# davidbau/rewriting

Measured on AMD Instinct MI355X. Metric: images/sec StyleGANv2-1024 fwd, higher is better.
Workload: dtype f32 (conv operands split into exact f16 pairs from 32x32 up, f32 accumulate); 1 GPU; stylegan2-1024 generator forward (FFHQ-1024 architecture); batch_per_gpu=64, mconv=seq, weights=synthetic seed 0, parallelism=seeds partitioned per rank, no collective, matrix_mode=split, direct_sums=auto

## Files before the change

### rewriting_amd/csrc/rw_dconv.hip

```cpp
#include "rw_common.h"
#include <stdlib.h>
typedef float dc_f32x4 __attribute__((ext_vector_type(4)));
typedef float dc_f32x2 __attribute__((ext_vector_type(2)));
typedef unsigned dc_u32x4 __attribute__((ext_vector_type(4)));
typedef int dc_i32x4 __attribute__((ext_vector_type(4)));
typedef _Float16 dc_f16x2 __attribute__((ext_vector_type(2)));
typedef _Float16 dc_f16x8 __attribute__((ext_vector_type(8)));

struct DconvProblem {
  const float* x; const unsigned char* wp; float* y;
  const float* style; const float* demod; const float* noise; const float* noise_w; const float* bias; int act;
  const float* post;
  const float* rgb_weight; const float* rgb_style; const float* rgb_bias; const float* rgb_skip; float* rgb_out;
  float rgb_scale;
  int batch, in_ch, out_ch, h, w;
  int tiles_x, tiles_y, o_tiles;
  int strided;
  float w_scale;
  float u_inv;
  const float* x_amax; float* y_amax;
};

#ifndef DC_ABL
#define DC_ABL 0
// ... 59 lines not shown
  constexpr int BUFB = NPIX * 64;
  constexpr int VCH = 32 * WM;
  __shared__ __attribute__((aligned(16))) unsigned char Ls[2 * BUFB];
  __shared__ __attribute__((aligned(16))) float St[512];
  __shared__ float Ct[2][VCH];
  __shared__ float Cr[3][(RGB || RGBP) ? 32 * WM : 1];
  __shared__ float Red[4];

  const int tid = threadIdx.x, lane = tid & 63;
  const int wave = __builtin_amdgcn_readfirstlane(tid >> 6);
  const int wm = wave / WN, wn = wave % WN;
  const int lk = lane >> 4, lt = lane & 15;

  const int local = dc_xcd_remap(blockIdx.x, gridDim.x);
  const int ot = local % p.o_tiles;
  int pg = local / p.o_tiles;
  const int tx = pg % p.tiles_x; pg /= p.tiles_x;
  const int ty = pg % p.tiles_y;
  const int ib = pg / p.tiles_y;
  const int y0 = ty * TR, x0 = tx * 32;
  const int64_t hw = (int64_t)p.h * p.w;
  const int NC = p.in_ch >> 4, T = 9 * NC;
  const int real_ch = UP ? p.out_ch >> 2 : p.out_ch;

  float in_scale, out_scale;
  {
    float smax = p.style ? 0.f : 1.f;
    if (p.style)
      for (int i = tid; i < p.in_ch; i += 256) smax = fmaxf(smax, fabsf(p.style[(int64_t)ib * p.in_ch + i]));
    smax = rw_wave_max(smax);
    if (lane == 0) Red[wave] = smax;
    __syncthreads();
    smax = fmaxf(fmaxf(Red[0], Red[1]), fmaxf(Red[2], Red[3]));
    const float am = rw_bound_load(p.x_amax) * smax;
    int e = (int)((__float_as_uint(am) >> 23) & 0xff) - 126;
    e = e < -100 ? -100 : (e > 100 ? 100 : e);
    in_scale = __uint_as_float((unsigned)(127 + 14 - e) << 23);
    out_scale = __uint_as_float((unsigned)(127 + e - 14) << 23) * p.u_inv;
  }
  const float gain = p.act ? 1.4142135623730951f : 1.f, slope = p.act ? 0.2f : 1.f;
  for (int i = tid; i < p.in_ch; i += 256) St[i] = (p.style ? p.style[(int64_t)ib * p.in_ch + i] : 1.0f) * in_scale;
  if (tid < VCH) {
    const int o = UP ? 16 * ot + (tid & 15) : ot * VCH + tid;
    Ct[0][tid] = (p.demod ? p.demod[(int64_t)ib * real_ch + o] * p.w_scale : p.w_scale) * out_scale * gain;
    Ct[1][tid] = p.act ? p.bias[o] * gain : 0.f;
    if (RGB || RGBP) {
      const float sr = p.rgb_scale * p.rgb_style[(int64_t)ib * p.out_ch + o];
#pragma unroll
      for (int cc = 0; cc < 3; ++cc) Cr[cc][tid] = sr * p.rgb_weight[cc * p.out_ch + o];
    }
  }
  const float noise_wg = p.noise ? p.noise_w[0] * gain : 0.f;
  __syncthreads();

  const __amdgpu_buffer_rsrc_t xsrc = __builtin_amdgcn_make_buffer_rsrc(
      const_cast<float*>(p.x + (int64_t)ib * p.in_ch * hw), 0, (int)((int64_t)p.in_ch * hw * 4), 0x00020000);
  const int hw4 = (int)hw * 4;
  int xoff[SI], loff[SI];
#pragma unroll
  for (int s = 0; s < SI; ++s) {
    const int pi = 64 * s + lane;
    const int r = pi / DC_PW, cc = pi - r * DC_PW;
    const int iy = y0 - 1 + r, ix = x0 - 1 + cc;
    const bool ok = pi < NPIX && iy >= 0 && iy < p.h && ix >= 0 && ix < p.w;
    xoff[s] = ok ? (iy * p.w + ix) * 4 : 0x7fffffff;
    loff[s] = pi < NPIX ? pi * 64 + ((wave ^ dc_swz(cc)) << 4) : -1;
  }
  constexpr int SH = (SI + 1) / 2;
  float raw[SH][4];
  auto stage_load = [&](int c, auto half_tag) __attribute__((always_inline)) {
    constexpr int S0 = decltype(half_tag)::value ? SH : 0, S1 = decltype(half_tag)::value ? SI : SH;
    const int s0 = (16 * c + 4 * wave) * hw4;
#pragma unroll
    for (int s = S0; s < S1; ++s)
#pragma unroll
      for (int k = 0; k < 4; ++k)
        raw[s - S0][k] = (DC_ABL & 1) ? 1.f : __uint_as_float(__builtin_amdgcn_raw_buffer_load_b32(xsrc, xoff[s], s0 + k * hw4, 0));
  };
  auto stage_store = [&](int c, int buf, auto half_tag) __attribute__((always_inline)) {
    constexpr int S0 = decltype(half_tag)::value ? SH : 0, S1 = decltype(half_tag)::value ? SI : SH;
    const dc_f32x4 sv = *reinterpret_cast<const dc_f32x4*>(&St[16 * c + 4 * wave]);
    unsigned char* dst = Ls + buf * BUFB;
#pragma unroll
    for (int s = S0; s < S1; ++s) {
      const float (&rw)[4] = raw[s - S0];
      const float v0 = rw[0] * sv[0], v1 = rw[1] * sv[1], v2 = rw[2] * sv[2], v3 = rw[3] * sv[3];
      const dc_f16x2 h01 = __builtin_convertvector(dc_f32x2{v0, v1}, dc_f16x2);
      const dc_f16x2 h23 = __builtin_convertvector(dc_f32x2{v2, v3}, dc_f16x2);
      float r0, r1, r2, r3;
      asm("v_fma_mix_f32 %0, -%1, 1.0, %2 op_sel_hi:[1,0,0]" : "=v"(r0) : "v"(h01), "v"(v0));
      asm("v_fma_mix_f32 %0, -%1, 1.0, %2 op_sel:[1,0,0] op_sel_hi:[1,0,0]" : "=v"(r1) : "v"(h01), "v"(v1));
      asm("v_fma_mix_f32 %0, -%1, 1.0, %2 op_sel_hi:[1,0,0]" : "=v"(r2) : "v"(h23), "v"(v2));
      asm("v_fma_mix_f32 %0, -%1, 1.0, %2 op_sel:[1,0,0] op_sel_hi:[1,0,0]" : "=v"(r3) : "v"(h23), "v"(v3));
      const dc_f16x2 l01 = __builtin_convertvector(dc_f32x2{r0, r1}, dc_f16x2);
      const dc_f16x2 l23 = __builtin_convertvector(dc_f32x2{r2, r3}, dc_f16x2);
      const dc_f16x8 word = {h01[0], h01[1], h23[0], h23[1], l01[0], l01[1], l23[0], l23[1]};
      if (loff[s] >= 0) *reinterpret_cast<dc_f16x8*>(dst + loff[s]) = word;
    }
  };

  const int vb0 = ot * (2 * WM) + 2 * wm;
  const unsigned char* wbase = p.wp + (int64_t)vb0 * T * 1024 + lane * 8;
  dc_f16x8 W[3][2][2];
  dc_f32x2 Wc[3][2][2];
  auto wload = [&](int ky, int t) __attribute__((always_inline)) {
#pragma unroll
    for (int ob = 0; ob < 2; ++ob)
#pragma unroll
      for (int part = 0; part < 2; ++part) {
        if (DC_ABL & 4) Wc[ky][ob][part] = dc_f32x2{1.f, 1.f};
        else Wc[ky][ob][part] = *reinterpret_cast<const dc_f32x2*>(wbase + ((int64_t)ob * T + t) * 1024 + part * 512);
      }
  };
  auto wexpand = [&](int ky) __attribute__((always_inline)) {
#pragma unroll
    for (int ob = 0; ob < 2; ++ob) {
      W[ky][ob][0] = dc_expand(Wc[ky][ob][0]);
      if (DC_PRODUCTS == 4 || ky == 2) W[ky][ob][1] = dc_expand(Wc[ky][ob][1]);
      else if (ky == 1) W[0][ob][1] = dc_pair(Wc[0][ob][1], Wc[1][ob][1]);
    }
  };

  dc_f32x4 acc[2][8];
#pragma unroll
  for (int ob = 0; ob < 2; ++ob)
#pragma unroll
    for (int pb = 0; pb < 8; ++pb) acc[ob][pb] = dc_f32x4{0.f, 0.f, 0.f, 0.f};

  unsigned bbase[3];
#pragma unroll
  for (int kx = 0; kx < 3; ++kx) {
    const int cc = lt + kx;
    bbase[kx] = (unsigned)((4 * wn * DC_PW + cc) * 64 + ((lk ^ dc_swz(cc)) << 4));
  }
  auto bread = [&](const unsigned char* lb, int kx, int idx) __attribute__((always_inline)) {
    return *reinterpret_cast<const dc_f16x8*>(lb + bbase[kx] + ((idx >> 1) * DC_PW + 16 * (idx & 1)) * 64);
  };

  auto chunk = [&](int c, auto last_tag) __attribute__((always_inline)) {
    constexpr bool LAST = decltype(last_tag)::value != 0;
    const int buf = c & 1;
    const unsigned char* lb = Ls + buf * BUFB;
    if (!LAST) stage_load(c + 1, rw_int<0>());
    dc_f16x8 bcur = bread(lb, 0, 0);
    dc_f16x8 bprev[2] = {bcur, bcur};
#pragma unroll
    for (int kx = 0; kx < 3; ++kx) {
      const bool more = !LAST || kx < 2;
      const int tn = kx < 2 ? 9 * c + kx + 1 : 9 * (c + 1);
#pragma unroll
      for (int idx = 0; idx < 12; ++idx) {
        const int r = idx >> 1, half = idx & 1;
        if (half == 0 && r < 3) wexpand(r);
        dc_f16x8 bnext = bcur;
        if (idx + 1 < 12) bnext = bread(lb, kx, idx + 1);
        else if (kx < 2) bnext = bread(lb, kx + 1, 0);
#pragma unroll
        for (int ky = 0; ky < 3; ++ky) {
          const int pr = r - ky;
          if (pr < 0 || pr > 3) continue;
          const int pb = 2 * pr + half;
          if (DC_ABL & 2) { asm volatile("" :: "v"(bcur), "v"(W[ky][0][0]), "v"(W[ky][0][1]), "v"(W[ky][1][0]), "v"(W[ky][1][1])); continue; }
          acc[0][pb] = __builtin_amdgcn_mfma_f32_16x16x32_f16(bcur, W[ky][0][0], acc[0][pb], 0, 0, 0);
          acc[1][pb] = __builtin_amdgcn_mfma_f32_16x16x32_f16(bcur, W[ky][1][0], acc[1][pb], 0, 0, 0);
          if (DC_PRODUCTS == 4 || ky == 2) {
            acc[0][pb] = __builtin_amdgcn_mfma_f32_16x16x32_f16(bcur, W[ky][0][1], acc[0][pb], 0, 0, 0);
            acc[1][pb] = __builtin_amdgcn_mfma_f32_16x16x32_f16(bcur, W[ky][1][1], acc[1][pb], 0, 0, 0);
          }
        }
        if (DC_PRODUCTS == 3 && r >= 1 && r <= 4 && !(DC_ABL & 2)) {
          const int pb = 2 * (r - 1) + half;
          const dc_f16x8 hh = dc_pair(bprev[half], bcur);
          acc[0][pb] = __builtin_amdgcn_mfma_f32_16x16x32_f16(hh, W[0][0][1], acc[0][pb], 0, 0, 0);
          acc[1][pb] = __builtin_amdgcn_mfma_f32_16x16x32_f16(hh, W[0][1][1], acc[1][pb], 0, 0, 0);
        }
        bprev[half] = bcur;
        __builtin_amdgcn_sched_barrier(0);
        if (more && half == 1 && r >= 3) wload(r - 3, tn + 3 * (r - 3));
        bcur = bnext;
      }
      if (!LAST && kx == 0) {
        stage_store(c + 1, buf ^ 1, rw_int<0>());
        stage_load(c + 1, rw_int<1>());
      }
      __builtin_amdgcn_sched_barrier(0);
    }
    if (!LAST) {
      stage_store(c + 1, buf ^ 1, rw_int<1>());
      __syncthreads();
    }
  };

  wload(0, 0);
  wload(1, 3);
  wload(2, 6);
  stage_load(0, rw_int<0>());
  stage_store(0, 0, rw_int<0>());
  stage_load(0, rw_int<1>());
  stage_store(0, 0, rw_int<1>());
  __syncthreads();

  for (int c = 0; c + 1 < NC; ++c) chunk(c, rw_int<0>());
  chunk(NC - 1, rw_int<1>());
  if (DC_ABL & 8) { if (acc[0][0][0] != 12345.f) return; }

  float ymax = 0.f;
  if (MODE == 0 || RGBP) {
    const int oc = 16 * (2 * wm) + lt;
    const float sc[2] = {Ct[0][oc], Ct[0][oc + 16]}, bs[2] = {Ct[1][oc], Ct[1][oc + 16]};
    float* yb = p.y + ((int64_t)ib * p.out_ch + ot * VCH + oc) * hw;
    float cr[2][3] = {{0.f, 0.f, 0.f}, {0.f, 0.f, 0.f}};
    float* rb = nullptr;
    if (RGBP) {
#pragma unroll
      for (int ob = 0; ob < 2; ++ob)
#pragma unroll
        for (int cc = 0; cc < 3; ++cc) cr[ob][cc] = Cr[cc][oc + 16 * ob];
      rb = p.rgb_out + (((int64_t)(ot * WM + wm) * p.batch + ib) * 3 + (lt < 3 ? lt : 0)) * hw;
    }
#pragma unroll
    for (int pb = 0; pb < 8; ++pb) {
      const int64_t pix = (int64_t)(y0 + 4 * wn + (pb >> 1)) * p.w + x0 + 16 * (pb & 1) + 4 * lk;
      dc_f32x4 nz = {0.f, 0.f, 0.f, 0.f};
      if (p.noise) nz = *reinterpret_cast<const dc_f32x4*>(p.noise + (int64_t)ib * hw + pix) * noise_wg;
      dc_f32x4 v[2];
#pragma unroll
      for (int ob = 0; ob < 2; ++ob) {
#pragma unroll
        for (int j = 0; j < 4; ++j) {
          const float u = acc[ob][pb][j] * sc[ob] + nz[j] + bs[ob];
          v[ob][j] = fmaxf(u, u * slope);
          ymax = fmaxf(ymax, fabsf(v[ob][j]));
        }
        *reinterpret_cast<dc_f32x4*>(yb + (int64_t)(16 * ob) * hw + pix) = v[ob];
      }
      if (RGBP) {
        dc_f32x4 sum[3];
#pragma unroll
        for (int j = 0; j < 4; ++j)
#pragma unroll
          for (int cc = 0; cc < 3; ++cc) sum[cc][j] = dc_row_sum(v[0][j] * cr[0][cc] + v[1][j] * cr[1][cc]);
        if (lt < 3) *reinterpret_cast<dc_f32x4*>(rb + pix) = lt == 0 ? sum[0] : (lt == 1 ? sum[1] : sum[2]);
      }
    }
  } else if (UP) {
    const float sc = Ct[0][lt], bs = Ct[1][lt];
    const int ch = 16 * ot + lt;
    const float post = p.post ? p.post[(int64_t)ib * real_ch + ch] : 1.f;
    const int W2 = 2 * p.w;
    const int64_t hw2 = 4 * hw;
    float* yb = p.y + ((int64_t)ib * real_ch + ch) * hw2;
#pragma unroll
    for (int pb = 0; pb < 8; ++pb) {
      const int64_t pix = (int64_t)(2 * (y0 + 4 * wn + (pb >> 1)) + wm) * W2 + 2 * (x0 + 16 * (pb & 1) + 4 * lk);
      dc_f32x4 n0 = {0.f, 0.f, 0.f, 0.f}, n1 = n0;
      if (p.noise) {
        const float* np = p.noise + (int64_t)ib * hw2 + pix;
        n0 = *reinterpret_cast<const dc_f32x4*>(np) * noise_wg;
        n1 = *reinterpret_cast<const dc_f32x4*>(np + 4) * noise_wg;
      }
      dc_f32x4 q0 = {acc[0][pb][0], acc[1][pb][0], acc[0][pb][1], acc[1][pb][1]};
      dc_f32x4 q1 = {acc[0][pb][2], acc[1][pb][2], acc[0][pb][3], acc[1][pb][3]};
#pragma unroll
      for (int k = 0; k < 4; ++k) {
        const float u0 = q0[k] * sc + n0[k] + bs, u1 = q1[k] * sc + n1[k] + bs;
        q0[k] = fmaxf(u0, u0 * slope) * post; q1[k] = fmaxf(u1, u1 * slope) * post;
        ymax = fmaxf(ymax, fmaxf(fabsf(q0[k]), fabsf(q1[k])));
      }
      *reinterpret_cast<dc_f32x4*>(yb + pix) = q0;
      *reinterpret_cast<dc_f32x4*>(yb + pix + 4) = q1;
    }
  } else {
    const float sc[2] = {Ct[0][lt], Ct[0][lt + 16]}, bs[2] = {Ct[1][lt], Ct[1][lt + 16]};
    float cr[2][3];
#pragma unroll
    for (int ob = 0; ob < 2; ++ob)
#pragma unroll
      for (int cc = 0; cc < 3; ++cc) cr[ob][cc] = Cr[cc][lt + 16 * ob];
#pragma unroll
    for (int pb = 0; pb < 8; ++pb) {
      const int64_t pix = (int64_t)(y0 + 4 * wn + (pb >> 1)) * p.w + x0 + 16 * (pb & 1) + 4 * lk;
      dc_f32x4 nz = {0.f, 0.f, 0.f, 0.f};
      if (p.noise) nz = *reinterpret_cast<const dc_f32x4*>(p.noise + (int64_t)ib * hw + pix) * noise_wg;
      dc_f32x4 sum[3];
#pragma unroll
      for (int j = 0; j < 4; ++j) {
        float u0 = acc[0][pb][j] * sc[0] + nz[j] + bs[0], u1 = acc[1][pb][j] * sc[1] + nz[j] + bs[1];
        u0 = fmaxf(u0, u0 * slope); u1 = fmaxf(u1, u1 * slope);
#pragma unroll
        for (int cc = 0; cc < 3; ++cc) sum[cc][j] = dc_row_sum(u0 * cr[0][cc] + u1 * cr[1][cc]);
      }
      if (lt < 3) {
        const dc_f32x4 mine = lt == 0 ? sum[0] : (lt == 1 ? sum[1] : sum[2]);
        const int64_t off = ((int64_t)ib * 3 + lt) * hw + pix;
        dc_f32x4 o4 = mine + (p.rgb_bias ? p.rgb_bias[lt] : 0.f);
        if (p.rgb_skip) o4 += *reinterpret_cast<const dc_f32x4*>(p.rgb_skip + off);
        *reinterpret_cast<dc_f32x4*>(p.rgb_out + off) = o4;
      }
    }
  }
  if (!RGB && p.y_amax) rw_bound_store_wave(p.y_amax, rw_wave_max(ymax));
}

template <int MODE, int WM, int MW, int NL, int WC>
__device__ __forceinline__ void dconv_ws_body(const DconvProblem& p) {
  constexpr bool UP = MODE == 1, RGB = MODE == 2, RGBP = MODE == 3, PLAIN = MODE == 0 || MODE == 3;
  static_assert(!RGB || WM == 1, "ToRGB: one wave holds all out-channels of its pixels");
  static_assert(!UP || WM == 2, "UP: the wave pairs are the two row phases");
  constexpr int WN = MW / WM, WR = WN / WC, TR = 4 * WR, PR = TR + 2, TC = 32 * WC, PW = TC + 2;
  static_assert(WR * WC == WN && WR >= 1, "strips tile the workgroup's pixels");
  constexpr int QW = 4 / NL, NLL = 64 * NL;
  constexpr int NPIX = PR * PW, BUFB = NPIX * 64;
  constexpr int IPR = TC / 4 + 2, NITEM = PR * IPR, SI = (NITEM + 63) / 64;
  constexpr int VCH = 32 * WM;
  constexpr int WBUF = 2 * WM * 9 * 1024;
  __shared__ __attribute__((aligned(16))) unsigned char Ls[2 * BUFB];
  __shared__ __attribute__((aligned(16))) unsigned char Wl[2 * WBUF];
  __shared__ float Ct[2][2][VCH];
  __shared__ float Cr[2][3][VCH];
  __shared__ float Po[2][16];

  const int tid = threadIdx.x, lane = tid & 63;
  const int wave = __builtin_amdgcn_readfirstlane(tid >> 6);
  const int64_t hw = (int64_t)p.h * p.w;
  const int NC = p.in_ch >> 4, T = 9 * NC;
  const int real_ch = UP ? p.out_ch >> 2 : p.out_ch;
  const float gain = p.act ? 1.4142135623730951f : 1.f, slope = p.act ? 0.2f : 1.f;

  const int64_t total = (int64_t)p.batch * p.tiles_y * p.tiles_x * p.o_tiles;
  const int per = (int)((total + gridDim.x - 1) / gridDim.x);
  const int bx = p.strided ? dc_xcd_remap(blockIdx.x, gridDim.x) : blockIdx.x;
  const int t0 = p.strided ? 0 : bx * per;
  const int t1 = p.strided ? (int)((total - bx + gridDim.x - 1) / gridDim.x)
                           : (int)((int64_t)t0 + per < total ? t0 + per : total);
  if (t0 >= t1) {
    if (!RGB && p.y_amax) rw_bound_store_wave(p.y_amax, 0.f);
    return;
  }
  const int N = (t1 - t0) * NC;
  const int t_mul = p.strided ? gridDim.x : 1, t_add = p.strided ? bx : 0;
  auto decode = [&](int pos, int& ot, int& tx, int& ty, int& ib) __attribute__((always_inline)) {
    const int tile = pos * t_mul + t_add;
    ot = tile % p.o_tiles;
    int pg = tile / p.o_tiles;
    tx = pg % p.tiles_x; pg /= p.tiles_x;
    ty = pg % p.tiles_y;
    ib = pg / p.tiles_y;
  };
  auto lds_barrier = [&]() __attribute__((always_inline)) {
    asm volatile("" ::: "memory");
    __builtin_amdgcn_s_waitcnt(0xC07F);
    __builtin_amdgcn_s_barrier();
    asm volatile("" ::: "memory");
  };

  if (wave >= MW) {
    const int g2 = QW * (wave - MW), lid = (wave - MW) * 64 + lane;
    const float xam = rw_bound_load(p.x_amax);
    const int hw4 = (int)hw * 4;
    int loff[SI];
#pragma unroll
    for (int s = 0; s < SI; ++s) {
      const int it = 64 * s + lane;
      const int r = it / IPR, j = it - r * IPR;
      loff[s] = it < NITEM ? (r * PW + 4 * j - 3) * 64 : -1000000;
    }
    int l_tile = t0, l_c = 0, l_ib = -1, l_ot = 0, l_y0 = 0, l_x0 = 0;
    float in_scale = 1.f, out_scale = 1.f;
    int xoff[SI];
    __amdgpu_buffer_rsrc_t xsrc = __builtin_amdgcn_make_buffer_rsrc(const_cast<float*>(p.x), 0, 0, 0x00020000);
    dc_f32x4 raw[QW][SI][4];
    float psv[QW][4];
    float a_demod = 1.f, a_bias = 0.f, a_rgb = 0.f, a_post = 1.f, a_oscale = 1.f, a_iscale = 1.f;
    float a_crw[3] = {0.f, 0.f, 0.f};
    bool a_first = false;
    int a_par = 0;
    float crw[3] = {0.f, 0.f, 0.f};
    if (RGB && lid < 32) {
#pragma unroll
      for (int cc = 0; cc < 3; ++cc) crw[cc] = p.rgb_weight[cc * p.out_ch + lid] * p.rgb_scale;
    }

    float sv[QW][4];
    int l_s0 = 0;
    const unsigned char* l_wsrc = p.wp;
    auto setup = [&]() __attribute__((always_inline)) {
      if (l_tile >= t1) { l_tile = t1 - 1; l_c = NC - 1; }
      a_first = l_c == 0;
      if (l_c == 0) {
        int tx, ty, ib;
        decode(l_tile, l_ot, tx, ty, ib);
        l_y0 = ty * TR; l_x0 = tx * TC;
        if (ib != l_ib) {
          l_ib = ib;
          float smax = 0.f;
          for (int i = lane; i < p.in_ch; i += 64) smax = fmaxf(smax, fabsf(p.style[(int64_t)ib * p.in_ch + i]));
          smax = rw_wave_max(smax);
          const float am = xam * smax;
          int e = (int)((__float_as_uint(am) >> 23) & 0xff) - 126;
          e = e < -100 ? -100 : (e > 100 ? 100 : e);
          in_scale = __uint_as_float((unsigned)(127 + 14 - e) << 23);
          out_scale = __uint_as_float((unsigned)(127 + e - 14) << 23) * p.u_inv;
          xsrc = __builtin_amdgcn_make_buffer_rsrc(const_cast<float*>(p.x + (int64_t)ib * p.in_ch * hw), 0,
                                                   (int)((int64_t)p.in_ch * hw * 4), 0x00020000);
        }
#pragma unroll
        for (int s = 0; s < SI; ++s) {
          const int it = 64 * s + lane;
          const int r = it / IPR, j = it - r * IPR;
          const int iy = l_y0 - 1 + r, ix = l_x0 - 4 + 4 * j;
          const bool ok = it < NITEM && iy >= 0 && iy < p.h && ix >= 0 && ix < p.w;
          xoff[s] = ok ? (iy * p.w + ix) * 4 : 0x7ffffff0;
        }
        a_par = (l_tile - t0) & 1;
        a_oscale = out_scale;
        if (lid < VCH) {
          const int o = UP ? 16 * l_ot + (lid & 15) : l_ot * VCH + lid;
          a_demod = p.demod ? p.demod[(int64_t)l_ib * real_ch + o] : 1.f;
          a_bias = p.act ? p.bias[o] : 0.f;
          if (RGB || RGBP) a_rgb = p.rgb_style[(int64_t)l_ib * p.out_ch + o];
          if (RGBP) {
#pragma unroll
            for (int cc = 0; cc < 3; ++cc) a_crw[cc] = p.rgb_weight[cc * p.out_ch + o] * p.rgb_scale;
          }
          if (UP && lid < 16 && p.post) a_post = p.post[(int64_t)l_ib * real_ch + o];
        }
      }
#pragma unroll
      for (int q = 0; q < QW; ++q)
#pragma unroll
        for (int k = 0; k < 4; ++k) psv[q][k] = p.style[(int64_t)l_ib * p.in_ch + 16 * l_c + 4 * (g2 + q) + k];
      a_iscale = in_scale;
      l_s0 = (16 * l_c + 4 * g2) * hw4;
      l_wsrc = p.wp + ((int64_t)(l_ot * (2 * WM) + (wave - MW)) * T + 9 * l_c) * 1024;
      if (++l_c == NC) { l_c = 0; ++l_tile; }
    };
    static_assert(NL == 2 * WM && SI == 3, "wave j stages weight block j, three tap pieces per pixel piece");
    dc_f32x4 wraw[SI][3];
    auto request_s = [&](int s) __attribute__((always_inline)) {
#pragma unroll
      for (int q = 0; q < QW; ++q)
#pragma unroll
        for (int k = 0; k < 4; ++k) {
          if (DC_ABL & 1) raw[q][s][k] = dc_f32x4{1.f, 1.f, 1.f, 1.f};
          else raw[q][s][k] = __builtin_bit_cast(dc_f32x4, __builtin_amdgcn_raw_buffer_load_b128(xsrc, xoff[s], l_s0 + (4 * q + k) * hw4, 0));
        }
#pragma unroll
      for (int k = 0; k < 3; ++k) {
        if (DC_ABL & 4) wraw[s][k] = dc_f32x4{1.f, 1.f, 1.f, 1.f};
        else wraw[s][k] = *reinterpret_cast<const dc_f32x4*>(l_wsrc + (3 * s + k) * 1024 + lane * 16);
      }
    };
    auto tables = [&]() __attribute__((always_inline)) {
#pragma unroll
      for (int q = 0; q < QW; ++q)
#pragma unroll
        for (int k = 0; k < 4; ++k) sv[q][k] = psv[q][k] * a_iscale;
      if (a_first) {
        if (lid < VCH) {
          Ct[a_par][0][lid] = a_demod * p.w_scale * a_oscale * gain;
          Ct[a_par][1][lid] = a_bias * gain;
          if (RGB || RGBP) {
#pragma unroll
            for (int cc = 0; cc < 3; ++cc) Cr[a_par][cc][lid] = a_rgb * (RGBP ? a_crw[cc] : crw[cc]);
          }
          if (UP && lid < 16) Po[a_par][lid] = a_post;
        }
      }
    };
    auto deliver_s = [&](int buf, int s) __attribute__((always_inline)) {
      unsigned char* dst = Ls + buf * BUFB;
      unsigned char* wdst = Wl + buf * WBUF + (wave - MW) * 9216 + lane * 16;
#pragma unroll
      for (int k = 0; k < 3; ++k) *reinterpret_cast<dc_f32x4*>(wdst + (3 * s + k) * 1024) = wraw[s][k];
      const int it = 64 * s + lane;
      const int j = it % IPR;
#pragma unroll
      for (int q = 0; q < QW; ++q)
#pragma unroll
        for (int e = 0; e < 4; ++e) {
          const float v0 = raw[q][s][0][e] * sv[q][0], v1 = raw[q][s][1][e] * sv[q][1], v2 = raw[q][s][2][e] * sv[q][2],
                      v3 = raw[q][s][3][e] * sv[q][3];
          const dc_f16x2 h01 = __builtin_convertvector(dc_f32x2{v0, v1}, dc_f16x2);
          const dc_f16x2 h23 = __builtin_convertvector(dc_f32x2{v2, v3}, dc_f16x2);
          float r0, r1, r2, r3;
          asm("v_fma_mix_f32 %0, -%1, 1.0, %2 op_sel_hi:[1,0,0]" : "=v"(r0) : "v"(h01), "v"(v0));
          asm("v_fma_mix_f32 %0, -%1, 1.0, %2 op_sel:[1,0,0] op_sel_hi:[1,0,0]" : "=v"(r1) : "v"(h01), "v"(v1));
          asm("v_fma_mix_f32 %0, -%1, 1.0, %2 op_sel_hi:[1,0,0]" : "=v"(r2) : "v"(h23), "v"(v2));
          asm("v_fma_mix_f32 %0, -%1, 1.0, %2 op_sel:[1,0,0] op_sel_hi:[1,0,0]" : "=v"(r3) : "v"(h23), "v"(v3));
          const dc_f16x2 l01 = __builtin_convertvector(dc_f32x2{r0, r1}, dc_f16x2);
          const dc_f16x2 l23 = __builtin_convertvector(dc_f32x2{r2, r3}, dc_f16x2);
          const dc_f16x8 word = {h01[0], h01[1], h23[0], h23[1], l01[0], l01[1], l23[0], l23[1]};
          const int cc = 4 * j - 3 + e;
          if (it < NITEM && cc >= 0 && cc < PW)
            *reinterpret_cast<dc_f16x8*>(dst + loff[s] + e * 64 + (((g2 + q) ^ dc_swz(cc)) << 4)) = word;
        }
    };

    setup();
#pragma unroll
    for (int s = 0; s < SI; ++s) request_s(s);
    tables();
    __builtin_amdgcn_sched_barrier(0);
    setup();
#pragma unroll
    for (int s = 0; s < SI; ++s) { deliver_s(0, s); __builtin_amdgcn_sched_barrier(0); request_s(s); __builtin_amdgcn_sched_barrier(0); }
    lds_barrier();
#if DC_PROF
    unsigned long long pt_del = 0, pt_req = 0, pt_bar = 0, pt_all = DC_T();
#endif
    for (int n = 0; n < N; ++n) {
#if DC_PROF
      const unsigned long long ta = DC_T();
#endif
      tables();
      __builtin_amdgcn_sched_barrier(0);
      setup();
#if DC_PROF
      const unsigned long long tb = DC_T();
#endif
#pragma unroll
      for (int s = 0; s < SI; ++s) { deliver_s((n + 1) & 1, s); __builtin_amdgcn_sched_barrier(0); request_s(s); __builtin_amdgcn_sched_barrier(0); }
#if DC_PROF
      const unsigned long long tc = DC_T();
#endif
      lds_barrier();
#if DC_PROF
      const unsigned long long td = DC_T();
      pt_del += tb - ta; pt_req += tc - tb; pt_bar += td - tc;
#endif
    }
#if DC_PROF
    if (wave == MW && lane == 0 && (blockIdx.x == 0 || blockIdx.x == 100)) {
      unsigned long long* o = dc_prof + (blockIdx.x == 0 ? 0 : 16);
      o[8] = DC_T() - pt_all; o[9] = pt_del; o[10] = pt_req; o[11] = pt_bar; o[12] = N;
    }
#endif
    if (!RGB && p.y_amax) rw_bound_store_wave(p.y_amax, 0.f);
    return;
  }

  const int wm = wave / WN, wn = wave % WN, wr = wn / WC, wc = wn % WC;
  const int lk = lane >> 4, lt = lane & 15;
  unsigned bbase[3];
#pragma unroll
  for (int kx = 0; kx < 3; ++kx) {
    const int cc = lt + kx;
    bbase[kx] = (unsigned)((4 * wr * PW + 32 * wc + cc) * 64 + ((lk ^ dc_swz(cc)) << 4));
  }
  auto bread = [&](const unsigned char* lb, int kx, int idx) __attribute__((always_inline)) {
    return *reinterpret_cast<const dc_f16x8*>(lb + bbase[kx] + ((idx >> 1) * PW + 16 * (idx & 1)) * 64);
  };
  dc_f16x8 W[3][2];
  dc_f32x2 Wc[3][2];
  auto wread = [&](const unsigned char* wb, int kx, int part) __attribute__((always_inline)) {
#pragma unroll
    for (int ky = 0; ky < 3; ++ky)
#pragma unroll
      for (int ob = 0; ob < 2; ++ob) {
        if (DC_ABL & 4) Wc[ky][ob] = dc_f32x2{1.f, 1.f};
        else Wc[ky][ob] = *reinterpret_cast<const dc_f32x2*>(wb + ((2 * wm + ob) * 9 + 3 * ky + kx) * 1024 + part * 512 + lane * 8);
      }
  };
  const float noise_wg = p.noise ? p.noise_w[0] * gain : 0.f;
  dc_f32x4 nzp[PLAIN ? 8 : 1];
  dc_f32x4 acc[2][8];
#pragma unroll
  for (int ob = 0; ob < 2; ++ob)
#pragma unroll
    for (int pb = 0; pb < 8; ++pb) acc[ob][pb] = dc_f32x4{0.f, 0.f, 0.f, 0.f};
  float ymax = 0.f;
  float rgb_b[3] = {0.f, 0.f, 0.f};
  if (RGB && p.rgb_bias) { rgb_b[0] = p.rgb_bias[0]; rgb_b[1] = p.rgb_bias[1]; rgb_b[2] = p.rgb_bias[2]; }

  int tile = t0, c = 0;
  int ot, tx, ty, ib;
  decode(tile, ot, tx, ty, ib);
  lds_barrier();

#if DC_PROF
  unsigned long long pt_mm = 0, pt_bar = 0, pt_epi = 0, pt_all = DC_T();
#endif
  for (int n = 0; n < N; ++n) {
#if DC_PROF
    const unsigned long long ta = DC_T();
#endif
    const unsigned char* lb = Ls + (n & 1) * BUFB;
    const unsigned char* wb = Wl + (n & 1) * WBUF;
    if (PLAIN && c == NC - 1 && p.noise) {
      const float* np = p.noise + (int64_t)ib * hw + (int64_t)(ty * TR + 4 * wr) * p.w + tx * TC + 32 * wc + 4 * lk;
#pragma unroll
      for (int pb = 0; pb < 8; ++pb) nzp[pb] = *reinterpret_cast<const dc_f32x4*>(np + (int64_t)(pb >> 1) * p.w + 16 * (pb & 1));
    }
    dc_f16x8 bq[3];
    wread(wb, 0, 0);
    bq[0] = bread(lb, 0, 0);
    bq[1] = bread(lb, 0, 1);
    dc_f16x8 bprev[2] = {bq[0], bq[1]};
#pragma unroll
    for (int hs = 0; hs < 6; ++hs) {
      const int kx = hs >> 1, part = hs & 1;
#pragma unroll
      for (int ob = 0; ob < 2; ++ob) {
        if (DC_PRODUCTS == 4 || part == 0) {
#pragma unroll
          for (int ky = 0; ky < 3; ++ky) W[ky][ob] = dc_expand(Wc[ky][ob]);
        } else {
          W[0][ob] = dc_pair(Wc[0][ob], Wc[1][ob]);
          W[2][ob] = dc_expand(Wc[2][ob]);
        }
      }
      __builtin_amdgcn_sched_barrier(0);
      if (hs + 1 < 6) wread(wb, (hs + 1) >> 1, (hs + 1) & 1);
      __builtin_amdgcn_sched_barrier(0);
#pragma unroll
      for (int idx = 0; idx < 12; ++idx) {
        const int r = idx >> 1, half = idx & 1;
        const dc_f16x8 b = bq[idx % 3];
        if (idx + 2 < 12) bq[(idx + 2) % 3] = bread(lb, kx, idx + 2);
        else if (hs < 5) bq[(idx + 2) % 3] = bread(lb, (hs + 1) >> 1, idx + 2 - 12);
        if (DC_PRODUCTS == 4 || part == 0) {
#pragma unroll
          for (int ky = 0; ky < 3; ++ky) {
            const int pr = r - ky;
            if (pr < 0 || pr > 3) continue;
            const int pb = 2 * pr + half;
            if (DC_ABL & 2) { asm volatile("" :: "v"(b), "v"(W[ky][0]), "v"(W[ky][1])); continue; }
            acc[0][pb] = __builtin_amdgcn_mfma_f32_16x16x32_f16(b, W[ky][0], acc[0][pb], 0, 0, 0);
            acc[1][pb] = __builtin_amdgcn_mfma_f32_16x16x32_f16(b, W[ky][1], acc[1][pb], 0, 0, 0);
          }
        } else if (DC_ABL & 2) {
          asm volatile("" :: "v"(b), "v"(W[0][0]), "v"(W[0][1]), "v"(W[2][0]), "v"(W[2][1]));
        } else {
          if (r >= 1 && r <= 4) {
            const int pb = 2 * (r - 1) + half;
            const dc_f16x8 hh = dc_pair(bprev[half], b);
            acc[0][pb] = __builtin_amdgcn_mfma_f32_16x16x32_f16(hh, W[0][0], acc[0][pb], 0, 0, 0);
            acc[1][pb] = __builtin_amdgcn_mfma_f32_16x16x32_f16(hh, W[0][1], acc[1][pb], 0, 0, 0);
          }
          if (r >= 2) {
            const int pb = 2 * (r - 2) + half;
            acc[0][pb] = __builtin_amdgcn_mfma_f32_16x16x32_f16(b, W[2][0], acc[0][pb], 0, 0, 0);
            acc[1][pb] = __builtin_amdgcn_mfma_f32_16x16x32_f16(b, W[2][1], acc[1][pb], 0, 0, 0);
          }
          bprev[half] = b;
        }
        __builtin_amdgcn_sched_barrier(0);
      }
    }
#if DC_PROF
    const unsigned long long tb = DC_T();
#endif
    lds_barrier();
#if DC_PROF
    const unsigned long long tc = DC_T();
    pt_mm += tb - ta; pt_bar += tc - tb;
    if (c + 1 == NC) pt_epi -= tc;
#endif
    if (++c < NC) continue;
    c = 0;
    const int par = (tile - t0) & 1;
    const int y0 = ty * TR, x0 = tx * TC;
    if (!(DC_ABL & 8)) {
      if (PLAIN) {
        const int oc = 16 * (2 * wm) + lt;
        const float sc[2] = {Ct[par][0][oc], Ct[par][0][oc + 16]}, bs[2] = {Ct[par][1][oc], Ct[par][1][oc + 16]};
        float* yb = p.y + ((int64_t)ib * p.out_ch + ot * VCH + oc) * hw;
        float cr[2][3] = {{0.f, 0.f, 0.f}, {0.f, 0.f, 0.f}};
        float* rb = nullptr;
        if (RGBP) {
#pragma unroll
          for (int ob = 0; ob < 2; ++ob)
#pragma unroll
            for (int cc = 0; cc < 3; ++cc) cr[ob][cc] = Cr[par][cc][oc + 16 * ob];
          rb = p.rgb_out + (((int64_t)(ot * WM + wm) * p.batch + ib) * 3 + (lt < 3 ? lt : 0)) * hw;
        }
#pragma unroll
        for (int pb = 0; pb < 8; ++pb) {
          const int64_t pix = (int64_t)(y0 + 4 * wr + (pb >> 1)) * p.w + x0 + 32 * wc + 16 * (pb & 1) + 4 * lk;
          dc_f32x4 nz = {0.f, 0.f, 0.f, 0.f};
          if (p.noise) nz = nzp[pb] * noise_wg;
          dc_f32x4 v[2];
#pragma unroll
          for (int ob = 0; ob < 2; ++ob) {
#pragma unroll
            for (int j = 0; j < 4; ++j) {
              const float u = acc[ob][pb][j] * sc[ob] + nz[j] + bs[ob];
              v[ob][j] = fmaxf(u, u * slope);
              ymax = fmaxf(ymax, fabsf(v[ob][j]));
            }
            if (!(DC_ABL & 16)) *reinterpret_cast<dc_f32x4*>(yb + (int64_t)(16 * ob) * hw + pix) = v[ob];
          }
          if (RGBP) {
            dc_f32x4 sum[3];
#pragma unroll
            for (int j = 0; j < 4; ++j)
#pragma unroll
              for (int cc = 0; cc < 3; ++cc) sum[cc][j] = dc_row_sum(v[0][j] * cr[0][cc] + v[1][j] * cr[1][cc]);
            if (lt < 3 && !(DC_ABL & 16)) *reinterpret_cast<dc_f32x4*>(rb + pix) = lt == 0 ? sum[0] : (lt == 1 ? sum[1] : sum[2]);
          }
        }
      } else if (UP) {
        const float sc = Ct[par][0][lt], bs = Ct[par][1][lt];
        const int ch = 16 * ot + lt;
        const float post = Po[par][lt];
        const int W2 = 2 * p.w;
        float* yb = p.y + ((int64_t)ib * real_ch + ch) * (4 * hw);
#pragma unroll
        for (int pb = 0; pb < 8; ++pb) {
          const int orow = 2 * (4 * wr + (pb >> 1)) + wm, ocol = 2 * (32 * wc + 16 * (pb & 1) + 4 * lk);
          const int64_t pix = (int64_t)(2 * y0 + orow) * W2 + 2 * x0 + ocol;
          dc_f32x4 n0 = {0.f, 0.f, 0.f, 0.f}, n1 = n0;
          if (p.noise) {
            const float* np = p.noise + (int64_t)ib * (4 * hw) + pix;
            n0 = *reinterpret_cast<const dc_f32x4*>(np) * noise_wg;
            n1 = *reinterpret_cast<const dc_f32x4*>(np + 4) * noise_wg;
          }
          dc_f32x4 q0 = {acc[0][pb][0], acc[1][pb][0], acc[0][pb][1], acc[1][pb][1]};
          dc_f32x4 q1 = {acc[0][pb][2], acc[1][pb][2], acc[0][pb][3], acc[1][pb][3]};
#pragma unroll
          for (int k = 0; k < 4; ++k) {
            const float u0 = q0[k] * sc + n0[k] + bs, u1 = q1[k] * sc + n1[k] + bs;
            q0[k] = fmaxf(u0, u0 * slope) * post; q1[k] = fmaxf(u1, u1 * slope) * post;
            ymax = fmaxf(ymax, fmaxf(fabsf(q0[k]), fabsf(q1[k])));
          }
          if (!(DC_ABL & 16)) {
            *reinterpret_cast<dc_f32x4*>(yb + pix) = q0;
            *reinterpret_cast<dc_f32x4*>(yb + pix + 4) = q1;
          }
        }
      } else {
        const float sc[2] = {Ct[par][0][lt], Ct[par][0][lt + 16]}, bs[2] = {Ct[par][1][lt], Ct[par][1][lt + 16]};
        float cr[2][3];
#pragma unroll
        for (int ob = 0; ob < 2; ++ob)
#pragma unroll
          for (int cc = 0; cc < 3; ++cc) cr[ob][cc] = Cr[par][cc][lt + 16 * ob];
#pragma unroll
        for (int pb = 0; pb < 8; ++pb) {
          const int64_t pix = (int64_t)(y0 + 4 * wr + (pb >> 1)) * p.w + x0 + 32 * wc + 16 * (pb & 1) + 4 * lk;
          dc_f32x4 nz = {0.f, 0.f, 0.f, 0.f};
          if (p.noise) nz = *reinterpret_cast<const dc_f32x4*>(p.noise + (int64_t)ib * hw + pix) * noise_wg;
          dc_f32x4 sum[3];
#pragma unroll
          for (int j = 0; j < 4; ++j) {
            float u0 = acc[0][pb][j] * sc[0] + nz[j] + bs[0], u1 = acc[1][pb][j] * sc[1] + nz[j] + bs[1];
            u0 = fmaxf(u0, u0 * slope); u1 = fmaxf(u1, u1 * slope);
#pragma unroll
            for (int cc = 0; cc < 3; ++cc) sum[cc][j] = dc_row_sum(u0 * cr[0][cc] + u1 * cr[1][cc]);
          }
          if (lt < 3) {
            const dc_f32x4 mine = lt == 0 ? sum[0] : (lt == 1 ? sum[1] : sum[2]);
            const int64_t off = ((int64_t)ib * 3 + lt) * hw + pix;
            dc_f32x4 o4 = mine + (lt == 0 ? rgb_b[0] : (lt == 1 ? rgb_b[1] : rgb_b[2]));
            if (p.rgb_skip) o4 += *reinterpret_cast<const dc_f32x4*>(p.rgb_skip + off);
            *reinterpret_cast<dc_f32x4*>(p.rgb_out + off) = o4;
          }
        }
      }
    }
#pragma unroll
    for (int ob = 0; ob < 2; ++ob)
#pragma unroll
      for (int pb = 0; pb < 8; ++pb) acc[ob][pb] = dc_f32x4{0.f, 0.f, 0.f, 0.f};
    if (++tile < t1) decode(tile, ot, tx, ty, ib);
#if DC_PROF
    pt_epi += DC_T();
#endif
  }
#if DC_PROF
  if (wave == 0 && lane == 0 && (blockIdx.x == 0 || blockIdx.x == 100)) {
    unsigned long long* o = dc_prof + (blockIdx.x == 0 ? 0 : 16);
    o[0] = DC_T() - pt_all; o[1] = pt_mm; o[2] = pt_bar; o[3] = pt_epi; o[4] = N;
  }
#endif
  if (!RGB && p.y_amax) rw_bound_store_wave(p.y_amax, rw_wave_max(ymax));
}

__global__ void __launch_bounds__(768, 3) dconv_ws_w2_kernel(const DconvProblem p) { dconv_ws_body<0, 2, 8, 4, 2>(p); }
__global__ void __launch_bounds__(768, 3) dconv_ws_up_kernel(const DconvProblem p) { dconv_ws_body<1, 2, 8, 4, 2>(p); }
__global__ void __launch_bounds__(768, 3) dconv_ws_w2_rgbp_kernel(const DconvProblem p) { dconv_ws_body<3, 2, 8, 4, 2>(p); }
__global__ void __launch_bounds__(384, 2) dconv_ws_rgb_kernel(const DconvProblem p) { dconv_ws_body<2, 1, 4, 2, 2>(p); }

__global__ void __launch_bounds__(256, 2) dconv_w1_kernel(const DconvProblem p) { dconv_body<0, 1>(p); }
__global__ void __launch_bounds__(256, 2) dconv_w2_kernel(const DconvProblem p) { dconv_body<0, 2>(p); }
__global__ void __launch_bounds__(256, 2) dconv_w4_kernel(const DconvProblem p) { dconv_body<0, 4>(p); }
__global__ void __launch_bounds__(256, 2) dconv_up_kernel(const DconvProblem p) { dconv_body<1, 2>(p); }
__global__ void __launch_bounds__(256, 2) dconv_rgb_kernel(const DconvProblem p) { dconv_body<2, 1>(p); }
__global__ void __launch_bounds__(256, 2) dconv_w1_rgbp_kernel(const DconvProblem p) { dconv_body<3, 1>(p); }
__global__ void __launch_bounds__(256, 2) dconv_w2_rgbp_kernel(const DconvProblem p) { dconv_body<3, 2>(p); }
__global__ void __launch_bounds__(256, 2) dconv_w4_rgbp_kernel(const DconvProblem p) { dconv_body<3, 4>(p); }

template <int PASS, bool UP>
__global__ void __launch_bounds__(256) pack_dconv_kernel(const float* __restrict__ w, const float* __restrict__ k4,
                                                         unsigned char* __restrict__ wp, float* __restrict__ trailer,
                                                         int vch, int in_ch, float su, float* __restrict__ bound) {
  const int64_t total = (int64_t)vch * in_ch;
  const int NC = in_ch >> 4, T = 9 * NC;
  float m = 0.f;
  for (int64_t idx = (int64_t)blockIdx.x * blockDim.x + threadIdx.x; idx < total; idx += (int64_t)gridDim.x * blockDim.x) {
    const int i = (int)(idx % in_ch), v = (int)(idx / in_ch);
    const int vb = v >> 4, n = v & 15;
    float h[9];
    if (UP) {
      const int ot = vb >> 2, py = (vb >> 1) & 1, px = vb & 1;
      const float* g = w + ((int64_t)(16 * ot + n) * in_ch + i) * 9;
#pragma unroll
      for (int a = 0; a < 3; ++a)
#pragma unroll
        for (int b = 0; b < 3; ++b) {
          const int ty = 2 - 2 * a + py, tx = 2 - 2 * b + px;
          float sum = 0.f;
#pragma unroll
          for (int c = 0; c < 4; ++c)
#pragma unroll
            for (int d = 0; d < 4; ++d) {
              const int ky = ty - 1 + c, kx = tx - 1 + d;
              if (ky >= 0 && ky < 3 && kx >= 0 && kx < 3) sum += k4[(3 - c) * 4 + (3 - d)] * g[3 * ky + kx];
            }
          h[3 * a + b] = sum;
        }
    } else {
      const float* g = w + ((int64_t)v * in_ch + i) * 9;
#pragma unroll
      for (int t = 0; t < 9; ++t) h[t] = g[t];
    }
    if (PASS == 1) {
#pragma unroll
      for (int t = 0; t < 9; ++t) m = fmaxf(m, fabsf(h[t]));
      continue;
    }
    const int c = i >> 4, g4 = (i & 15) >> 2, k = i & 3, lane = 16 * g4 + n;
    _Float16* dst = reinterpret_cast<_Float16*>(wp + ((int64_t)vb * T + 9 * c) * 1024) + lane * 4 + k;
#pragma unroll
    for (int t = 0; t < 9; ++t) {
      const float u = h[t] * su;
      const _Float16 hi = (_Float16)u;
      const _Float16 lo = (_Float16)(u - (float)hi);
      _Float16* d = dst + t * 512;
      d[0] = hi;
      d[256] = lo;
    }
  }
  __shared__ float red[4];
// ... 225 lines not shown
```

Measured before the change: 1581 images/sec.

## Use 32x32x16 MFMA path for plain modulated convolutions

Adds a compute path for plain (non-upsampling, non-RGB) convolution modes that uses 32x32x16 f16 MFMA instructions in place of the previous 16-wide tile formulation. Producer waves write weights and activation hi/lo halves into LDS in a new layout with a new swizzle matched to the 32-lane operand pattern. The epilogue is rewritten for the 32x32 accumulator layout, including vectorised scale and bias reads and fused ToRGB partial sums. The larger MFMA shape is meant to raise matrix throughput per instruction and reuse operands better, at the cost of new LDS layouts, more accumulator registers and possible bank conflicts.

After: 1602 images/sec, median of 6. 1.01x the previous value.

```diff
diff --git a/rewriting_amd/csrc/rw_dconv.hip b/rewriting_amd/csrc/rw_dconv.hip
--- a/rewriting_amd/csrc/rw_dconv.hip
+++ b/rewriting_amd/csrc/rw_dconv.hip
@@ -385,9 +385,15 @@
   if (!RGB && p.y_amax) rw_bound_store_wave(p.y_amax, rw_wave_max(ymax));
 }
 
+#ifndef DC_MFMA32
+#define DC_MFMA32 1
+#endif
+__device__ __forceinline__ int dc_swz32(int cc) { return (cc >> 2) & 3; }
+
 template <int MODE, int WM, int MW, int NL, int WC>
 __device__ __forceinline__ void dconv_ws_body(const DconvProblem& p) {
   constexpr bool UP = MODE == 1, RGB = MODE == 2, RGBP = MODE == 3, PLAIN = MODE == 0 || MODE == 3;
+  constexpr bool M32 = PLAIN && DC_MFMA32;
   static_assert(!RGB || WM == 1, "ToRGB: one wave holds all out-channels of its pixels");
   static_assert(!UP || WM == 2, "UP: the wave pairs are the two row phases");
   constexpr int WN = MW / WM, WR = WN / WC, TR = 4 * WR, PR = TR + 2, TC = 32 * WC, PW = TC + 2;
@@ -399,8 +405,8 @@
   constexpr int WBUF = 2 * WM * 9 * 1024;
   __shared__ __attribute__((aligned(16))) unsigned char Ls[2 * BUFB];
   __shared__ __attribute__((aligned(16))) unsigned char Wl[2 * WBUF];
-  __shared__ float Ct[2][2][VCH];
-  __shared__ float Cr[2][3][VCH];
+  __shared__ __attribute__((aligned(16))) float Ct[2][2][VCH];
+  __shared__ __attribute__((aligned(16))) float Cr[2][3][VCH];
   __shared__ float Po[2][16];
 
   const int tid = threadIdx.x, lane = tid & 63;
@@ -553,9 +559,20 @@
     };
     auto deliver_s = [&](int buf, int s) __attribute__((always_inline)) {
       unsigned char* dst = Ls + buf * BUFB;
-      unsigned char* wdst = Wl + buf * WBUF + (wave - MW) * 9216 + lane * 16;
-#pragma unroll
-      for (int k = 0; k < 3; ++k) *reinterpret_cast<dc_f32x4*>(wdst + (3 * s + k) * 1024) = wraw[s][k];
+      if (M32) {
+        const int jw = wave - MW, lp = lane & 31, g = lp >> 3, m = 16 * (jw & 1) + 2 * (lp & 7);
+        unsigned char* wdst = Wl + buf * WBUF + ((jw >> 1) * 18 + (lane >> 5)) * 1024 + (32 * (g >> 1) + m) * 16 + 8 * (g & 1);
+#pragma unroll
+        for (int k = 0; k < 3; ++k) {
+          unsigned char* d = wdst + (3 * s + k) * 2048;
+          *reinterpret_cast<dc_f32x2*>(d) = dc_f32x2{wraw[s][k][0], wraw[s][k][1]};
+          *reinterpret_cast<dc_f32x2*>(d + 16) = dc_f32x2{wraw[s][k][2], wraw[s][k][3]};
+        }
+      } else {
+        unsigned char* wdst = Wl + buf * WBUF + (wave - MW) * 9216 + lane * 16;
+#pragma unroll
+        for (int k = 0; k < 3; ++k) *reinterpret_cast<dc_f32x4*>(wdst + (3 * s + k) * 1024) = wraw[s][k];
+      }
       const int it = 64 * s + lane;
       const int j = it % IPR;
 #pragma unroll
@@ -573,10 +590,21 @@
           asm("v_fma_mix_f32 %0, -%1, 1.0, %2 op_sel:[1,0,0] op_sel_hi:[1,0,0]" : "=v"(r3) : "v"(h23), "v"(v3));
           const dc_f16x2 l01 = __builtin_convertvector(dc_f32x2{r0, r1}, dc_f16x2);
           const dc_f16x2 l23 = __builtin_convertvector(dc_f32x2{r2, r3}, dc_f16x2);
-          const dc_f16x8 word = {h01[0], h01[1], h23[0], h23[1], l01[0], l01[1], l23[0], l23[1]};
           const int cc = 4 * j - 3 + e;
-          if (it < NITEM && cc >= 0 && cc < PW)
-            *reinterpret_cast<dc_f16x8*>(dst + loff[s] + e * 64 + (((g2 + q) ^ dc_swz(cc)) << 4)) = word;
+          if (M32) {
+            const int g = g2 + q, f = dc_swz32(cc);
+            unsigned char* d = dst + loff[s] + e * 64 + 8 * (g & 1);
+            if (it < NITEM && cc >= 0 && cc < PW) {
+              *reinterpret_cast<dc_f32x2*>(d + (((g >> 1) ^ f) << 4)) =
+                  dc_f32x2{__builtin_bit_cast(float, h01), __builtin_bit_cast(float, h23)};
+              *reinterpret_cast<dc_f32x2*>(d + (((2 + (g >> 1)) ^ f) << 4)) =
+                  dc_f32x2{__builtin_bit_cast(float, l01), __builtin_bit_cast(float, l23)};
+            }
+          } else {
+            const dc_f16x8 word = {h01[0], h01[1], h23[0], h23[1], l01[0], l01[1], l23[0], l23[1]};
+            if (it < NITEM && cc >= 0 && cc < PW)
+              *reinterpret_cast<dc_f16x8*>(dst + loff[s] + e * 64 + (((g2 + q) ^ dc_swz(cc)) << 4)) = word;
+          }
         }
     };
 
@@ -623,6 +651,132 @@
     return;
   }
 
+  if constexpr (M32) {
+    const int wm = wave / WN, wn = wave % WN, wr = wn / WC, wc = wn % WC;
+    const int lj = lane & 31, lh = lane >> 5;
+    unsigned pbase[3][2];
+#pragma unroll
+    for (int kx = 0; kx < 3; ++kx) {
+      const int cc = 32 * wc + kx + lj;
+#pragma unroll
+      for (int pc = 0; pc < 2; ++pc) pbase[kx][pc] = (unsigned)((4 * wr * PW + cc) * 64 + (((2 * pc + lh) ^ dc_swz32(cc)) << 4));
+    }
+    const unsigned wlane = (unsigned)(wm * 18 * 1024 + lane * 16);
+    auto pread = [&](const unsigned char* lb, int kx, int pc, int rr) __attribute__((always_inline)) {
+      return *reinterpret_cast<const dc_f16x8*>(lb + pbase[kx][pc] + rr * PW * 64);
+    };
+    auto wread = [&](const unsigned char* wb, int ky, int kx, int pc) __attribute__((always_inline)) {
+      return *reinterpret_cast<const dc_f16x8*>(wb + wlane + ((3 * ky + kx) * 2 + pc) * 1024);
+    };
+    const float noise_wg = p.noise ? p.noise_w[0] * gain : 0.f;
+    float nzp[4] = {0.f, 0.f, 0.f, 0.f};
+    rw_f32x16 acc[4];
+#pragma unroll
+    for (int pr = 0; pr < 4; ++pr) acc[pr] = rw_f32x16{};
+    float ymax = 0.f;
+
+    int tile = t0, c = 0;
+    int ot, tx, ty, ib;
+    decode(tile, ot, tx, ty, ib);
+    lds_barrier();
+    for (int n = 0; n < N; ++n) {
+      const unsigned char* lb = Ls + (n & 1) * BUFB;
+      const unsigned char* wb = Wl + (n & 1) * WBUF;
+      if (c == NC - 1 && p.noise) {
+        const float* np = p.noise + (int64_t)ib * hw + (int64_t)(ty * TR + 4 * wr) * p.w + tx * TC + 32 * wc + lj;
+#pragma unroll
+        for (int pr = 0; pr < 4; ++pr) nzp[pr] = np[(int64_t)pr * p.w];
+      }
+      dc_f16x8 W[3][2];
+      dc_f16x8 B[2][2];
+#pragma unroll
+      for (int ky = 0; ky < 3; ++ky)
+#pragma unroll
+        for (int pc = 0; pc < 2; ++pc) W[ky][pc] = wread(wb, ky, 0, pc);
+      B[0][0] = pread(lb, 0, 0, 0);
+      B[0][1] = pread(lb, 0, 1, 0);
+#pragma unroll
+      for (int kx = 0; kx < 3; ++kx) {
+#pragma unroll
+        for (int rr = 0; rr < 6; ++rr) {
+          const int cb = rr & 1;
+          if (rr < 5) {
+            B[cb ^ 1][0] = pread(lb, kx, 0, rr + 1);
+            B[cb ^ 1][1] = pread(lb, kx, 1, rr + 1);
+          } else if (kx < 2) {
+            B[cb ^ 1][0] = pread(lb, kx + 1, 0, 0);
+            B[cb ^ 1][1] = pread(lb, kx + 1, 1, 0);
+          }
+#pragma unroll
+          for (int prod = 0; prod < 3; ++prod)
+#pragma unroll
+            for (int ky = 0; ky < 3; ++ky) {
+              const int pr = rr - ky;
+              if (pr < 0 || pr > 3) continue;
+              acc[pr] = __builtin_amdgcn_mfma_f32_32x32x16_f16(W[ky][prod == 2], B[cb][prod == 1], acc[pr], 0, 0, 0);
+            }
+          __builtin_amdgcn_sched_barrier(0);
+          if (rr >= 3 && kx < 2) {
+            W[rr - 3][0] = wread(wb, rr - 3, kx + 1, 0);
+            W[rr - 3][1] = wread(wb, rr - 3, kx + 1, 1);
+          }
+          __builtin_amdgcn_sched_barrier(0);
+        }
+      }
+      lds_barrier();
+      if (++c < NC) continue;
+      c = 0;
+      const int par = (tile - t0) & 1;
+      const int hw4 = (int)hw * 4;
+      const int pix0 = (ty * TR + 4 * wr) * p.w + tx * TC + 32 * wc + lj;
+      const __amdgpu_buffer_rsrc_t ysrc = __builtin_amdgcn_make_buffer_rsrc(
+          p.y + ((int64_t)ib * p.out_ch + ot * VCH + 32 * wm) * hw, 0, 32 * hw4, 0x00020000);
+      const int ocb = 32 * wm + 4 * lh;
+#pragma unroll
+      for (int pr = 0; pr < 4; ++pr) {
+        const int yoff = (4 * lh * (int)hw + pix0 + pr * p.w) * 4;
+        const float nz = nzp[pr] * noise_wg;
+        float rs[3] = {0.f, 0.f, 0.f};
+#pragma unroll
+        for (int g4 = 0; g4 < 4; ++g4) {
+          const int oc = ocb + 8 * g4;
+          const dc_f32x4 sc = *reinterpret_cast<const dc_f32x4*>(&Ct[par][0][oc]);
+          const dc_f32x4 bs = *reinterpret_cast<const dc_f32x4*>(&Ct[par][1][oc]);
+          dc_f32x4 cr[3] = {};
+          if (RGBP) {
+#pragma unroll
+            for (int cc = 0; cc < 3; ++cc) cr[cc] = *reinterpret_cast<const dc_f32x4*>(&Cr[par][cc][oc]);
+          }
+#pragma unroll
+          for (int e = 0; e < 4; ++e) {
+            const float u = acc[pr][4 * g4 + e] * sc[e] + nz + bs[e];
+            const float v = fmaxf(u, u * slope);
+            ymax = fmaxf(ymax, fabsf(v));
+            __builtin_amdgcn_raw_buffer_store_b32(__builtin_bit_cast(unsigned, v), ysrc, yoff, (8 * g4 + e) * hw4, 0);
+            if (RGBP) {
+#pragma unroll
+              for (int cc = 0; cc < 3; ++cc) rs[cc] += v * cr[cc][e];
+            }
+          }
+        }
+        if (RGBP) {
+          const __amdgpu_buffer_rsrc_t rsrc = __builtin_amdgcn_make_buffer_rsrc(
+              p.rgb_out + ((int64_t)(ot * WM + wm) * p.batch + ib) * 3 * hw, 0, 3 * hw4, 0x00020000);
+          float t[3];
+#pragma unroll
+          for (int cc = 0; cc < 3; ++cc) t[cc] = rs[cc] + __shfl_xor(rs[cc], 32, 64);
+          const int roff = (pix0 + pr * p.w) * 4;
+          __builtin_amdgcn_raw_buffer_store_b32(__builtin_bit_cast(unsigned, lh ? t[1] : t[0]), rsrc, roff, lh * hw4, 0);
+          if (!lh) __builtin_amdgcn_raw_buffer_store_b32(__builtin_bit_cast(unsigned, t[2]), rsrc, roff, 2 * hw4, 0);
+        }
+      }
+#pragma unroll
+      for (int pr = 0; pr < 4; ++pr) acc[pr] = rw_f32x16{};
+      if (++tile < t1) decode(tile, ot, tx, ty, ib);
+    }
+    if (p.y_amax) rw_bound_store_wave(p.y_amax, rw_wave_max(ymax));
+    return;
+  }
   const int wm = wave / WN, wn = wave % WN, wr = wn / WC, wc = wn % WC;
   const int lk = lane >> 4, lt = lane & 15;
   unsigned bbase[3];
```
